# AutonomousVehicleLaboratory/vision_semantic_segmentation

Measured on AMD Instinct MI355X. Metric: fused frames/sec/GPU (1920x1080 + 120k pts) + max|dlog-odds| vs ref, higher is better.
Workload: dtype f16 hi+lo split, MX-FP4 correction passes, fp32 accumulate

## Files before the change

include/avl_hip.h:

```cpp
#ifndef AVL_HIP_H
#define AVL_HIP_H

#include <stdint.h>

#ifdef __cplusplus
extern "C" {
#endif

#define AVL_OK 0
#define AVL_E_ARG (-1)
#define AVL_E_HIP (-2)
#define AVL_E_UNSUPPORTED (-3)

#define AVL_F32 0
#define AVL_F64 1
#define AVL_BF16 2
#define AVL_F16 3

#define AVL_MAX_MAP_CLASSES 16

const char* avl_version(void);
int avl_last_error(char* buf, int len);


// ... 290 lines not shown
#define AVL_OP_SUBSAMPLE 10
#define AVL_OP_DWPW 11

#define AVL_OP_BOTTLENECK 12

typedef struct avl_seg_op {
    int32_t kind;
    int32_t dtype;
    const void* in;
    const void* in2;
    void* out;
    const void* weight;
    const float* bias;
    int32_t in_h, in_w, in_c, in_ld, in_rows;
    int32_t out_h, out_w, out_c, out_ld, out_rows;
    int32_t in2_ld;
    int32_t ksize, stride, pad, dil, groups;
    int32_t relu;
    int32_t out_f32;
    int32_t w_rows;
    int32_t w_layout;
    int32_t w_split;
    int32_t mx_flags;
    const void* in_lo;
    const void* in2_lo;
    void* out_lo;
    const void* w_mx;
    const void* in_mx;
    void* out_mx;
    const void* in2_mx;
    const void* in3;
    const void* in3_mx;
    int32_t in3_c, in3_ld;
    int32_t batch;
    int32_t bias_per_image;
    int32_t in_format;
    int32_t raw_batch;
    void* out2;
    void* out2_lo;
    int32_t out2_ld, n_split;
} avl_seg_op;

#define AVL_IN_U8_HWC 0
#define AVL_IN_F32_CHW 1

#define AVL_MX_IN_LO 1
#define AVL_MX_RES_LO 2
#define AVL_MX_OUT_LO 4

typedef struct avl_seg_plan avl_seg_plan;

int avl_seg_plan_create(const avl_seg_op* ops_host, int n_ops, avl_seg_plan** out_plan);
void avl_seg_plan_destroy(avl_seg_plan* plan);
int avl_seg_plan_run(avl_seg_plan* plan, void* stream);
int avl_seg_plan_capture(avl_seg_plan* plan, void* stream);
int avl_seg_plan_profile(avl_seg_plan* plan, void* stream, float* ms_host, double* flops_host, double* bytes_host);
int avl_seg_plan_num_ops(const avl_seg_plan* plan);
int avl_seg_plan_nonfinite(avl_seg_plan* plan, void* stream, unsigned long long* counts_host);

#define AVL_GEMM_PLAIN 0
#define AVL_GEMM_RING 1
#define AVL_GEMM_RING_MX 2
#define AVL_GEMM_MX_PIPE 3

typedef struct avl_gemm_route {
    int32_t kernel;
    int32_t dtype;
    int32_t tile_m, tile_n;
    int32_t wm, wn;
    int32_t mi;
    int32_t stages;
    int32_t nsub;
    int32_t io;
    int32_t ast;
    int32_t ext;
    int32_t late;
    int32_t launches;
    int32_t m_tiles, n_tiles;
    int32_t workgroups;
} avl_gemm_route;

int avl_seg_gemm_route(const avl_seg_op* op, avl_gemm_route* out);

#ifdef __cplusplus
}
#endif
#endif
```

vision_semantic_segmentation_amd/csrc/seg_conv.hip:

```cpp
#include "seg_types.h"
#include "seg_preprocess.h"

namespace avl {
namespace {

constexpr int kThreads = 256;

template <typename T, bool F32IN = false>
__global__ void __launch_bounds__(kThreads) k_stem(const unsigned char* __restrict__ img, int H, int W,
                                                  const float* __restrict__ w, const float* __restrict__ bias,
                                                  T* __restrict__ out, int OH, int OW, int out_ld) {
    const int idx = blockIdx.x * kThreads + threadIdx.x;
    if (idx >= OH * OW) return;
    img = image_base(img, (long long)H * W, F32IN ? 3 * (int)sizeof(float) : 3);
    out = image_base(out, (long long)OH * OW, out_ld);
    const int oy = idx / OW, ox = idx % OW;
    float acc[64];
#pragma unroll
    for (int c = 0; c < 64; ++c) acc[c] = bias[c];
    const float mean[3] = {0.485f, 0.456f, 0.406f}, stdv[3] = {0.229f, 0.224f, 0.225f};
    for (int ky = 0; ky < 7; ++ky) {
        const int iy = oy * 2 - 3 + ky;
        for (int kx = 0; kx < 7; ++kx) {
            const int ix = ox * 2 - 3 + kx;
// ... 358 lines not shown
    }
}

template <typename T>
__global__ void __launch_bounds__(kThreads) k_dwconv_split(const T* __restrict__ in, const T* __restrict__ in_lo, const float* __restrict__ w,
                                                          const float* __restrict__ bias, T* __restrict__ out, T* __restrict__ out_lo,
                                                          int H, int W, int C, int in_ld, int OH, int OW, int out_ld, int pad, int dil, int relu) {
    const int c8n = C / 8;
    const long long idx = (long long)blockIdx.x * kThreads + threadIdx.x;
    if (idx >= (long long)OH * OW * c8n) return;
    in = image_base(in, (long long)H * W, in_ld);
    in_lo = image_base(in_lo, (long long)H * W, in_ld);
    out = image_base(out, (long long)OH * OW, out_ld);
    out_lo = image_base(out_lo, (long long)OH * OW, out_ld);
    const int c8 = (int)(idx % c8n);
    const int pix = (int)(idx / c8n), oy = pix / OW, ox = pix % OW;
    float acc[8];
    {
        const float4 b0 = *reinterpret_cast<const float4*>(bias + c8 * 8), b1 = *reinterpret_cast<const float4*>(bias + c8 * 8 + 4);
        acc[0] = b0.x; acc[1] = b0.y; acc[2] = b0.z; acc[3] = b0.w; acc[4] = b1.x; acc[5] = b1.y; acc[6] = b1.z; acc[7] = b1.w;
    }
    float xv[9][8];
    bool ok[9];
#pragma unroll
    for (int t = 0; t < 9; ++t) {
        const int iy = oy - pad + (t / 3) * dil, ix = ox - pad + (t % 3) * dil;
        ok[t] = iy >= 0 && iy < H && ix >= 0 && ix < W;
        const long long o = ok[t] ? ((long long)iy * W + ix) * in_ld + c8 * 8 : (long long)c8 * 8;
        Vec8<T>::load(in + o, xv[t]);
        if (in_lo) {
            float l[8];
            Vec8<T>::load(in_lo + o, l);
#pragma unroll
            for (int i = 0; i < 8; ++i) xv[t][i] += l[i];
        }
    }
#pragma unroll
    for (int t = 0; t < 9; ++t) {
        const float4 w0 = *reinterpret_cast<const float4*>(w + t * C + c8 * 8), w1 = *reinterpret_cast<const float4*>(w + t * C + c8 * 8 + 4);
        const float wt[8] = {w0.x, w0.y, w0.z, w0.w, w1.x, w1.y, w1.z, w1.w};
#pragma unroll
        for (int i = 0; i < 8; ++i) acc[i] = fmaf(ok[t] ? xv[t][i] : 0.f, wt[i], acc[i]);
    }
    if (relu) {
#pragma unroll
        for (int i = 0; i < 8; ++i) acc[i] = fmaxf(acc[i], 0.f);
    }
    Vec8<T>::store(out + (long long)pix * out_ld + c8 * 8, acc);
    if (out_lo) {
#pragma unroll
        for (int i = 0; i < 8; ++i) acc[i] -= to_f32(from_f32<T>(acc[i]));
        Vec8<T>::store(out_lo + (long long)pix * out_ld + c8 * 8, acc);
    }
}

template <typename T>
__global__ void __launch_bounds__(kThreads) k_gap_partial(const T* __restrict__ in, int M, int C, int in_ld,
                                                         float* __restrict__ partial) {
    const int c8n = C / 8;
    const int G = gridDim.x;
    in = image_base(in, M, in_ld);
    partial = image_base(partial, G, C);
    for (int c8 = threadIdx.x; c8 < c8n; c8 += kThreads) {
        float s[8] = {0, 0, 0, 0, 0, 0, 0, 0};
        int r = blockIdx.x;
        for (; r + 3 * G < M; r += 4 * G) {
            float v0[8], v1[8], v2[8], v3[8];
            Vec8<T>::load(in + (long long)r * in_ld + c8 * 8, v0);
            Vec8<T>::load(in + (long long)(r + G) * in_ld + c8 * 8, v1);
            Vec8<T>::load(in + (long long)(r + 2 * G) * in_ld + c8 * 8, v2);
            Vec8<T>::load(in + (long long)(r + 3 * G) * in_ld + c8 * 8, v3);
#pragma unroll
            for (int i = 0; i < 8; ++i) s[i] += (v0[i] + v1[i]) + (v2[i] + v3[i]);
        }
        for (; r < M; r += G) {
            float v[8];
            Vec8<T>::load(in + (long long)r * in_ld + c8 * 8, v);
#pragma unroll
            for (int i = 0; i < 8; ++i) s[i] += v[i];
        }
        Vec8<float>::store(partial + (long long)blockIdx.x * C + c8 * 8, s);
    }
}
__global__ void __launch_bounds__(kThreads) k_gap_final(const float* __restrict__ partial, int G, int C, int M,
                                                       float* __restrict__ out, int out_ld) {
    __shared__ float red[8][32];
    const int cl = threadIdx.x & 31, sl = threadIdx.x >> 5;
    const int c = blockIdx.x * 32 + cl;
    partial = image_base(partial, G, C);
    out = image_base(out, 1, out_ld);
    float s = 0.f;
    if (c < C)
        for (int g = sl; g < G; g += 8) s += partial[(long long)g * C + c];
    red[sl][cl] = s;
    __syncthreads();
    if (sl == 0 && c < C) {
        float t = 0.f;
#pragma unroll
        for (int k = 0; k < 8; ++k) t += red[k][cl];
        out[c] = t / (float)M;
    }
}

__global__ void __launch_bounds__(kThreads) k_gemv(const float* __restrict__ in, const float* __restrict__ w,
                                                  const float* __restrict__ bias, float* __restrict__ out, int N, int K, int relu,
                                                  int in_ld, int out_ld) {
    const int n = blockIdx.x * (kThreads / 64) + (threadIdx.x >> 6);
    const int lane = threadIdx.x & 63;
    if (n >= N) return;
    in = image_base(in, 1, in_ld);
    out = image_base(out, 1, out_ld);
    const float* wr = w + (long long)n * K;
    float s0 = 0.f, s1 = 0.f, s2 = 0.f, s3 = 0.f;
    if ((K & 3) == 0 && (reinterpret_cast<uintptr_t>(wr) & 15) == 0 && (reinterpret_cast<uintptr_t>(in) & 15) == 0) {
#pragma unroll 8
        for (int k = lane * 4; k < K; k += 256) {
            const float4 a = *reinterpret_cast<const float4*>(wr + k), b = *reinterpret_cast<const float4*>(in + k);
            s0 = fmaf(a.x, b.x, s0); s1 = fmaf(a.y, b.y, s1); s2 = fmaf(a.z, b.z, s2); s3 = fmaf(a.w, b.w, s3);
        }
    } else {
        for (int k = lane; k < K; k += 64) s0 = fmaf(wr[k], in[k], s0);
    }
    float s = (s0 + s1) + (s2 + s3);
#pragma unroll
    for (int off = 32; off > 0; off >>= 1) s += __shfl_down(s, off);
    if (lane == 0) {
        s += bias ? bias[n] : 0.f;
        out[n] = relu ? fmaxf(s, 0.f) : s;
    }
}

__global__ void __launch_bounds__(kThreads) k_argmax(const float* __restrict__ logits, int M, int C, int ld,
                                                    unsigned char* __restrict__ out) {
    const int m = blockIdx.x * kThreads + threadIdx.x;
    if (m >= M) return;
    const float* p = logits + (long long)m * ld;
    float best = p[0];
    int bi = 0;
    for (int c = 1; c < C; ++c) {
        const float v = p[c];
        if (v > best || (v != v && best == best)) { best = v; bi = c; }
    }
    out[m] = (unsigned char)bi;
}

template <typename T>
__global__ void __launch_bounds__(kThreads) k_subsample(const T* __restrict__ in, int W, int C, int in_ld,
                                                       T* __restrict__ out, int H, int OH, int OW, int out_ld, int stride) {
    const int c8n = C / 8;
    const long long idx = (long long)blockIdx.x * kThreads + threadIdx.x;
    if (idx >= (long long)OH * OW * c8n) return;
    in = image_base(in, (long long)H * W, in_ld);
    out = image_base(out, (long long)OH * OW, out_ld);
    const int c8 = (int)(idx % c8n);
    const int pix = (int)(idx / c8n), oy = pix / OW, ox = pix % OW;
    float v[8];
    Vec8<T>::load(in + ((long long)(oy * stride) * W + ox * stride) * in_ld + c8 * 8, v);
    Vec8<T>::store(out + (long long)pix * out_ld + c8 * 8, v);
}

__global__ void __launch_bounds__(kThreads) k_preprocess(const unsigned char* __restrict__ bgr, int H, int W, PreParams q,
                                                        unsigned char* __restrict__ out, int OH, int OW) {
    const int idx = blockIdx.x * kThreads + threadIdx.x;
    if (idx >= OH * OW) return;
    int v[3];
    preprocessed_rgb(bgr, H, W, q.cam, q.factor, idx % OW, idx / OW, v);
#pragma unroll
    for (int c = 0; c < 3; ++c) out[3ll * idx + c] = (unsigned char)v[c];
}

struct AreaAxis { int s1, s2; float w_first, w_mid, w_last; };
__device__ __forceinline__ AreaAxis area_axis(int d, double scale, int ssize) {
    const double f1 = d * scale, f2 = f1 + scale;
    const double cell = fmin(scale, (double)ssize - f1);
    int s1 = (int)ceil(f1), s2 = (int)floor(f2);
    s2 = min(s2, ssize - 1);
// ... 46 lines not shown
                break;
            }
            hipLaunchKernelGGL(k_stem<T>, dim3(blocks_for((long long)op.out_h * op.out_w), 1, nimg), dim3(kThreads), 0, s,
                               static_cast<const unsigned char*>(op.in), op.in_h, op.in_w, w, op.bias, out, op.out_h, op.out_w,
                               op.out_ld);
            break;
        case AVL_OP_MAXPOOL:
            hipLaunchKernelGGL(k_maxpool<T>, dim3(blocks_for((long long)op.out_h * op.out_w * (op.in_c / 8)), 1, nimg), dim3(kThreads), 0, s,
                               in, op.in_h, op.in_w, op.in_c, op.in_ld, out, op.out_h, op.out_w, op.out_ld, static_cast<const T*>(op.in_lo),
                               static_cast<T*>(op.out_lo));
            break;
        case AVL_OP_GCONV: {
            const int cg = op.in_c / op.groups;
            const dim3 grid(blocks_for((long long)op.out_h * op.out_w), op.groups, nimg);
#define AVL_GCONV(CG)                                                                                                   \
    hipLaunchKernelGGL((k_gconv<T, CG>), grid, dim3(kThreads), 0, s, in, op.in_h, op.in_w, op.in_ld, w, op.bias, out, \
                       op.out_h, op.out_w, op.out_ld, op.stride, op.dil)
            if (cg == 4) AVL_GCONV(4);
            else if (cg == 8) AVL_GCONV(8);
            else if (cg == 16) AVL_GCONV(16);
            else if (cg == 32) AVL_GCONV(32);
            else if (cg == 2) AVL_GCONV(2);
            else return set_error(AVL_E_UNSUPPORTED, "grouped conv with %d channels per group", cg);
#undef AVL_GCONV
            break;
        }
        case AVL_OP_DWCONV: {
            if (op.ksize != 3) return launch_dwconv_k(op, s);
            if ((op.in_lo == nullptr) != (op.out_lo == nullptr) && !op.out_mx) {
                hipLaunchKernelGGL(k_dwconv_split<T>, dim3(blocks_for((long long)op.out_h * op.out_w * (op.in_c / 8)), 1, nimg), dim3(kThreads), 0, s,
                                   in, static_cast<const T*>(op.in_lo), w, op.bias, out, static_cast<T*>(op.out_lo), op.in_h, op.in_w,
                                   op.in_c, op.in_ld, op.out_h, op.out_w, op.out_ld, op.pad, op.dil, op.relu);
                break;
            }
            DwGeom g;
            g.H = op.in_h; g.W = op.in_w; g.C = op.in_c; g.in_ld = op.in_ld; g.OH = op.out_h; g.OW = op.out_w; g.out_ld = op.out_ld;
            g.pad = op.pad; g.dil = op.dil; g.relu = op.relu;
            g.gh = (op.out_h + op.dil - 1) / op.dil;
            g.gw = (op.out_w + op.dil - 1) / op.dil;
            const int chunks = op.in_c / 8;
            g.nchunk = chunks < 64 ? chunks : 64;
            while (chunks % g.nchunk) --g.nchunk;
            g.cl = kThreads / g.nchunk;
            g.cgroups = chunks / g.nchunk;
            const long long combs = (long long)op.dil * op.dil;
            g.band_w = g.gw; g.band_h = g.gh;
            if (op.dil == 1) {
                g.band_w = 2 * g.cl < g.gw ? 2 * g.cl : g.gw;
                g.band_h = g.gh < 16 ? g.gh : 16;
                const int nbx = (g.gw + g.band_w - 1) / g.band_w;
                while (g.band_h > 4 && (long long)g.cgroups * nbx * ((g.gh + g.band_h - 1) / g.band_h) < 512) g.band_h = (g.band_h + 1) / 2;
            }
            g.nbx = (g.gw + g.band_w - 1) / g.band_w;
            g.nby = (g.gh + g.band_h - 1) / g.band_h;
            g.units = (int)(combs * g.nby * g.nbx);
            const int target = 32 * g.cl, unit_px = g.band_h * g.band_w;
            g.upb = (op.dil == 1 || unit_px >= target) ? 1 : (target + unit_px - 1) / unit_px;
            const unsigned nblk = (unsigned)((g.units + g.upb - 1) / g.upb) * g.cgroups;
            if constexpr (sizeof(T) == 2) {
                if (op.in_lo && (op.out_lo || op.out_mx)) {
                    MxOut mx;
                    memset(&mx, 0, sizeof(mx));
                    if (op.out_mx) {
                        const auto o = mx_bundle(op.out_mx, op.out_rows, op.out_c);
                        mx.q[0] = o.q[0]; mx.s[0] = o.s[0];
                        if (op.out_lo || (op.mx_flags & AVL_MX_OUT_LO)) { mx.q[1] = o.q[1]; mx.s[1] = o.s[1]; }
                        mx.srows = o.srows; mx.ldq = o.ldq;
                    }
                    hipLaunchKernelGGL((k_dwconv<T, true>), dim3(nblk, 1, nimg), dim3(kThreads), 0, s, in, w, op.bias, out,
                                       static_cast<const T*>(op.in2), g, static_cast<const T*>(op.in_lo), static_cast<T*>(op.out_lo), mx);
                    break;
                }
            }
            hipLaunchKernelGGL((k_dwconv<T, false>), dim3(nblk, 1, nimg), dim3(kThreads), 0, s, in, w, op.bias, out,
                               static_cast<const T*>(op.in2), g, static_cast<const T*>(nullptr), static_cast<T*>(nullptr), MxOut());
            break;
        }
        case AVL_OP_BILINEAR:
            hipLaunchKernelGGL(k_bilinear<T>, dim3(blocks_for((long long)op.out_h * op.out_w * (op.in_c / 8)), 1, nimg), dim3(kThreads), 0, s,
                               in, static_cast<const T*>(op.in_lo), op.in_h, op.in_w, op.in_c, op.in_ld, out, static_cast<T*>(op.out_lo),
                               op.out_h, op.out_w, op.out_ld);
            break;
        case AVL_OP_GAP: {
            const int G = 256;
            float* partial = static_cast<float*>(const_cast<void*>(op.in2));
            hipLaunchKernelGGL(k_gap_partial<T>, dim3(G, 1, nimg), dim3(kThreads), 0, s, in, op.in_h * op.in_w, op.in_c, op.in_ld, partial);
            AVL_LAUNCH_CHECK();
            hipLaunchKernelGGL(k_gap_final, dim3((op.in_c + 31) / 32, 1, nimg), dim3(kThreads), 0, s, partial, G, op.in_c,
                               op.in_h * op.in_w, static_cast<float*>(op.out), op.out_ld);
            break;
        }
        case AVL_OP_SUBSAMPLE:
            hipLaunchKernelGGL(k_subsample<T>, dim3(blocks_for((long long)op.out_h * op.out_w * (op.in_c / 8)), 1, nimg), dim3(kThreads), 0, s,
                               in, op.in_w, op.in_c, op.in_ld, out, op.in_h, op.out_h, op.out_w, op.out_ld, op.stride);
            break;
        default:
            return set_error(AVL_E_ARG, "op kind %d is not a typed conv op", op.kind);
    }
    AVL_LAUNCH_CHECK();
    return AVL_OK;
}

}

int validate_conv_op(const avl_seg_op& op) {
    const int es = elem_size(op.dtype);
    AVL_REQUIRE(op.in && op.out, "op %d has NULL in/out", op.kind);
    AVL_REQUIRE(op.in_h > 0 && op.in_w > 0 && op.out_h > 0 && op.out_w > 0, "op %d has empty spatial dims", op.kind);
    const long long in_pix = (long long)op.in_h * op.in_w * op_batch(op), out_pix = (long long)op.out_h * op.out_w * op_batch(op);
    switch (op.kind) {
        case AVL_OP_STEM:
            if (op.in2 && op_batch(op) > 1 && !op.raw_batch)
                return set_error(AVL_E_UNSUPPORTED, "a pre-processing stem (in2 = camera block) takes one raw frame unless raw_batch = 1: batch %d",
                                 op.batch);
            AVL_REQUIRE(op.weight && op.bias && op.out_c == 64 && op.in_c == 3, "stem expects 3 -> 64 channels");
            if (op.stride == 4) {
                const int ch = (op.in_h + 6 - 7) / 2 + 1, cw = (op.in_w + 6 - 7) / 2 + 1;
                AVL_REQUIRE(is_half(op.dtype) && op.w_layout == 1, "a pooled stem (stride 4) is the MFMA kernel (16-bit, w_layout 1): dtype %d, w_layout %d",
                            op.dtype, op.w_layout);
                AVL_REQUIRE(!op.w_split && !op.out_lo, "a pooled stem (stride 4) writes one plane: w_split %d with%s out_lo", op.w_split, op.out_lo ? "" : "out");
                AVL_REQUIRE(op.out_h == (ch + 2 - 3) / 2 + 1 && op.out_w == (cw + 2 - 3) / 2 + 1, "pooled stem output size %d x %d (conv %d x %d)",
                            op.out_h, op.out_w, ch, cw);
                AVL_REQUIRE(reinterpret_cast<uintptr_t>(op.out) % 16 == 0, "pooled stem: unaligned output");
            } else
                AVL_REQUIRE(op.out_h == (op.in_h + 6 - 7) / 2 + 1 && op.out_w == (op.in_w + 6 - 7) / 2 + 1, "stem output size");
            AVL_REQUIRE(op.out_rows >= out_pix && op.out_ld >= 64 && (op.out_ld * es) % 16 == 0, "stem output buffer");
            AVL_REQUIRE(op.w_layout == 0 || (op.w_layout == 1 && is_half(op.dtype)), "stem weight layout %d", op.w_layout);
            if (op.in2) {
                AVL_REQUIRE(is_half(op.dtype) ? op.w_layout == 1 : (op.dtype == AVL_F32 && op.w_layout == 0),
                            "a pre-processing stem is the MFMA kernel (16-bit, w_layout 1) or the fp32 kernel (AVL_F32, w_layout 0): dtype %d, w_layout %d",
                            op.dtype, op.w_layout);
                AVL_REQUIRE(reinterpret_cast<uintptr_t>(op.in2) % 4 == 0, "stem camera block alignment: in2 (one block, or `batch` blocks of "
                            "AVL_STEM_CAMERA_BYTES with raw_batch) must be 4-byte aligned");
                const int nb = op_batch(op);
                AVL_REQUIRE(op.in2_ld > 0 && op.in_rows > 0 && op.in_rows % nb == 0 && (op.in_rows / nb) % op.in2_ld == 0,
                            "stem raw frame: in_rows %d is not batch %d * src_h * src_w for an integer src_h (in2_ld = src_w = %d)", op.in_rows, nb, op.in2_ld);
                const int src_w = op.in2_ld, src_h = op.in_rows / nb / op.in2_ld, f = src_w / op.in_w;
                AVL_REQUIRE(f >= 1 && op.in_w == src_w / f && op.in_h == src_h / f, "stem raw frame %dx%d does not scale to %dx%d by an integer factor",
                            src_h, src_w, op.in_h, op.in_w);
            } else {
                AVL_REQUIRE(op.in_rows >= in_pix, "stem input buffer");
            }
            return AVL_OK;
        case AVL_OP_GEMV:
            AVL_REQUIRE(op.dtype == AVL_F32, "gemv reads and writes fp32 vectors: dtype %d", op.dtype);
            AVL_REQUIRE(op.weight && op.in_c > 0 && op.out_c > 0, "gemv shapes");
            AVL_REQUIRE(op_batch(op) == 1 || (op.in_ld >= op.in_c && op.out_ld >= op.out_c), "batched gemv: vector strides in_ld %d / out_ld %d", op.in_ld, op.out_ld);
            return AVL_OK;
        case AVL_OP_ARGMAX:
            AVL_REQUIRE(op.dtype == AVL_F32, "argmax reads fp32 logits: dtype %d", op.dtype);
            AVL_REQUIRE(op.in_c > 0 && op.in_c <= 256 && op.in_ld >= op.in_c && op.in_rows >= in_pix && op.out_rows >= in_pix, "argmax shapes");
            return AVL_OK;
        case AVL_OP_GAP:
            AVL_REQUIRE(is_half(op.dtype) || op.dtype == AVL_F32, "gap dtype %d", op.dtype);
            AVL_REQUIRE(op.in2 && op.in_c % 8 == 0 && op.in_rows >= in_pix && op.in_ld >= op.in_c, "gap shapes / scratch");
            AVL_REQUIRE((op.in_ld * es) % 16 == 0, "gap in_ld");
            AVL_REQUIRE((reinterpret_cast<uintptr_t>(op.in) | reinterpret_cast<uintptr_t>(op.in2)) % 16 == 0, "gap input / scratch not 16-byte aligned");
            AVL_REQUIRE(op_batch(op) == 1 || op.out_ld >= op.in_c, "batched gap: out_ld %d", op.out_ld);
            return AVL_OK;
        default:
            break;
    }
    AVL_REQUIRE(is_half(op.dtype) || op.dtype == AVL_F32, "op %d dtype %d", op.kind, op.dtype);
    AVL_REQUIRE(op.in_c % 8 == 0 || (op.kind == AVL_OP_GCONV), "op %d: channels %d not a multiple of 8", op.kind, op.in_c);
    AVL_REQUIRE(op.in_rows >= in_pix && op.out_rows >= out_pix, "op %d: allocated rows too small", op.kind);
    AVL_REQUIRE(op.in_ld >= op.in_c && op.out_ld >= op.out_c, "op %d: leading dims", op.kind);
    AVL_REQUIRE((op.in_ld * es) % 16 == 0 && (op.out_ld * es) % 16 == 0, "op %d: row strides must be 16-byte multiples", op.kind);
    AVL_REQUIRE((reinterpret_cast<uintptr_t>(op.in) | reinterpret_cast<uintptr_t>(op.out)) % 16 == 0, "op %d: unaligned buffers", op.kind);
    if (op.out_mx && op.kind == AVL_OP_DWCONV && op.ksize == 3) {
        AVL_REQUIRE(op.dtype == AVL_F16 && op.in_lo && op.out_c % 256 == 0 && op.out_ld == op.out_c && (op.in_c / 8) % 4 == 0,
                    "dwconv: out_mx needs the split f16 form, channels %% 256 == 0 and a dense output");
// ... 95 lines not shown
```

vision_semantic_segmentation_amd/csrc/seg_stem_mfma.hip:

```cpp
#include "seg_types.h"
#include "seg_preprocess.h"

namespace avl {
namespace {

constexpr int S_TH = 8, S_TW = 32;
constexpr int ROW = 224;

template <typename HT>
struct StemArgs {
    const unsigned char* img;
    const HT* w;
    const float* bias;
    HT* out;
    HT* out_lo;
    int H, W, OH, OW, out_ld, tiles_x;
    int PH, PW;
    const PreCamera* cam;
    int srcH, srcW, factor;
};

template <typename HT, bool PRE, bool SPLIT = false, bool F32IN = false, bool POOL = false>
__global__ void __launch_bounds__(256) k_stem_mfma(StemArgs<HT> p) {
    typedef typename Half16<HT>::v8 v8;
// ... 168 lines not shown
                } else {
#pragma unroll
                    for (int i = 0; i < 8; ++i) al[i] = (HT)0.f;
                }
#pragma unroll
                for (int nj = 0; nj < 4; ++nj) {
                    const v8 wl = *reinterpret_cast<const v8*>(p.w + 4 * 6 * 16 * 32 + ((nj * 6 + st) * 16 + fr) * 32 + kq * 8);
                    acc[nj] = Half16<HT>::mfma(wf[nj][st], al, acc[nj]);
                    acc[nj] = Half16<HT>::mfma(wl, a, acc[nj]);
                }
            }
        }
        if constexpr (POOL) {
            if (sub * 16 + fr < NPOS) {
                float lo[8], hi[8];
#pragma unroll
                for (int r = 0; r < 4; ++r) {
                    lo[r] = fmaxf(acc[0][r] + bias[r], 0.f);
                    lo[4 + r] = fmaxf(acc[1][r] + bias[4 + r], 0.f);
                    hi[r] = fmaxf(acc[2][r] + bias[8 + r], 0.f);
                    hi[4 + r] = fmaxf(acc[3][r] + bias[12 + r], 0.f);
                }
                const int pos = sy * CTW + sx;
                HT* sp = stage + pos * 64;
                Vec8<HT>::store(sp + (((kq * 2) ^ (pos & 7)) << 3), lo);
                Vec8<HT>::store(sp + (((kq * 2 + 1) ^ (pos & 7)) << 3), hi);
            }
            continue;
        }
        const int oy = oy0 + sy, ox = ox0 + sx;
        if (oy < p.OH && ox < p.OW) {
            float lo[8], hi[8];
#pragma unroll
            for (int r = 0; r < 4; ++r) {
                lo[r] = fmaxf(acc[0][r] + bias[r], 0.f);
                lo[4 + r] = fmaxf(acc[1][r] + bias[4 + r], 0.f);
                hi[r] = fmaxf(acc[2][r] + bias[8 + r], 0.f);
                hi[4 + r] = fmaxf(acc[3][r] + bias[12 + r], 0.f);
            }
            HT* op = p.out + ((long long)oy * p.OW + ox) * p.out_ld + kq * 16;
            if constexpr (SPLIT) {
                float l0[8], l1[8];
#pragma unroll
                for (int r = 0; r < 8; ++r) {
                    const float h0 = (float)(HT)lo[r], h1 = (float)(HT)hi[r];
                    l0[r] = lo[r] - h0; l1[r] = hi[r] - h1;
                    lo[r] = h0; hi[r] = h1;
                }
                HT* ol = p.out_lo + ((long long)oy * p.OW + ox) * p.out_ld + kq * 16;
                Vec8<HT>::store(ol, l0);
                Vec8<HT>::store(ol + 8, l1);
            }
            Vec8<HT>::store(op, lo);
            Vec8<HT>::store(op + 8, hi);
        }
    }
    if constexpr (POOL) {
        __syncthreads();
        for (int i = tid; i < 4 * 16 * 8; i += 256) {
            const int c = i & 7, lpy = i >> 7, lpx = (i >> 3) & 15;
            const int py = ty * 4 + lpy, px = tx * 16 + lpx;
            if (py >= p.PH || px >= p.PW) continue;
            float m[8];
#pragma unroll
            for (int j = 0; j < 8; ++j) m[j] = -INFINITY;
            for (int ky = 0; ky < 3; ++ky) {
                const int cy = py * 2 - 1 + ky;
                if (cy < 0 || cy >= p.OH) continue;
                for (int kx = 0; kx < 3; ++kx) {
                    const int cx = px * 2 - 1 + kx;
                    if (cx < 0 || cx >= p.OW) continue;
                    const int pos = (lpy * 2 + ky) * CTW + lpx * 2 + kx;
                    float v[8];
                    Vec8<HT>::load(stage + pos * 64 + ((c ^ (pos & 7)) << 3), v);
#pragma unroll
                    for (int j = 0; j < 8; ++j) m[j] = fmaxf(m[j], v[j]);
                }
            }
            Vec8<HT>::store(p.out + ((long long)py * p.PW + px) * p.out_ld + c * 8, m);
        }
    }
}

}

template <typename HT>
int launch_stem_typed(const avl_seg_op& op, hipStream_t s) {
    StemArgs<HT> a;
    a.img = static_cast<const unsigned char*>(op.in);
    a.w = static_cast<const HT*>(op.weight);
    a.bias = op.bias;
    a.out = static_cast<HT*>(op.out);
    a.out_lo = static_cast<HT*>(op.out_lo);
    a.H = op.in_h; a.W = op.in_w; a.OH = op.out_h; a.OW = op.out_w; a.out_ld = op.out_ld;
    const bool pool = op.stride == 4;
    a.PH = op.out_h; a.PW = op.out_w;
    if (pool) { a.OH = (op.in_h + 6 - 7) / 2 + 1; a.OW = (op.in_w + 6 - 7) / 2 + 1; }
    a.tiles_x = pool ? (op.out_w + 15) / 16 : (op.out_w + S_TW - 1) / S_TW;
    const int tiles_y = pool ? (op.out_h + 3) / 4 : (op.out_h + S_TH - 1) / S_TH;
    a.cam = static_cast<const PreCamera*>(op.in2);
    a.srcW = op.in2_ld;
    a.srcH = op.in2_ld > 0 ? op.in_rows / op_batch(op) / op.in2_ld : 0;
    a.factor = op.in_w > 0 ? a.srcW / op.in_w : 1;
    const dim3 grid(a.tiles_x * tiles_y, 1, op_batch(op));
    if (pool) {
        if (op.in_format == AVL_IN_F32_CHW) hipLaunchKernelGGL((k_stem_mfma<HT, false, false, true, true>), grid, dim3(256), 0, s, a);
        else if (op.in2) hipLaunchKernelGGL((k_stem_mfma<HT, true, false, false, true>), grid, dim3(256), 0, s, a);
        else hipLaunchKernelGGL((k_stem_mfma<HT, false, false, false, true>), grid, dim3(256), 0, s, a);
    } else if (op.in_format == AVL_IN_F32_CHW) {
        if (op.w_split) {
            if (!op.out_lo) return set_error(AVL_E_ARG, "split stem (w_split = 1): out_lo is NULL");
            hipLaunchKernelGGL((k_stem_mfma<HT, false, true, true>), grid, dim3(256), 0, s, a);
        } else {
            hipLaunchKernelGGL((k_stem_mfma<HT, false, false, true>), grid, dim3(256), 0, s, a);
        }
    } else if (op.w_split) {
        if (!op.out_lo) return set_error(AVL_E_ARG, "split stem (w_split = 1): out_lo is NULL");
        if (op.in2)
            hipLaunchKernelGGL((k_stem_mfma<HT, true, true>), grid, dim3(256), 0, s, a);
        else
            hipLaunchKernelGGL((k_stem_mfma<HT, false, true>), dim3(a.tiles_x * tiles_y, 1, op_batch(op)), dim3(256), 0, s, a);
    } else if (op.in2)
        hipLaunchKernelGGL((k_stem_mfma<HT, true>), grid, dim3(256), 0, s, a);
    else
        hipLaunchKernelGGL((k_stem_mfma<HT, false>), dim3(a.tiles_x * tiles_y, 1, op_batch(op)), dim3(256), 0, s, a);
    AVL_LAUNCH_CHECK();
    return AVL_OK;
}

int launch_stem_mfma(const avl_seg_op& op, hipStream_t s) {
    return op.dtype == AVL_F16 ? launch_stem_typed<f16>(op, s) : launch_stem_typed<bf16>(op, s);
}

}
```

vision_semantic_segmentation_amd/network.py:

```python
import collections
import ctypes as C
import hashlib
import math

import numpy as np
import torch

from . import _lib

BN_EPS = 1e-5

OP_STEM, OP_MAXPOOL, OP_GEMM, OP_GCONV, OP_DWCONV, OP_BILINEAR, OP_GAP, OP_GEMV, OP_ARGMAX, OP_SUBSAMPLE, OP_DWPW, OP_BOTTLENECK = range(1, 13)
OP_NAMES = {1: "stem", 2: "maxpool", 3: "gemm", 4: "gconv", 5: "dwconv", 6: "bilinear", 7: "gap", 8: "gemv", 9: "argmax", 10: "subsample", 11: "dwpw",
            12: "bottleneck"}


class AvlSegOp(C.Structure):
    _fields_ = [
        ("kind", C.c_int32), ("dtype", C.c_int32),
        ("in_", C.c_void_p), ("in2", C.c_void_p), ("out", C.c_void_p), ("weight", C.c_void_p), ("bias", C.c_void_p),
        ("in_h", C.c_int32), ("in_w", C.c_int32), ("in_c", C.c_int32), ("in_ld", C.c_int32), ("in_rows", C.c_int32),
        ("out_h", C.c_int32), ("out_w", C.c_int32), ("out_c", C.c_int32), ("out_ld", C.c_int32), ("out_rows", C.c_int32),
        ("in2_ld", C.c_int32),
        ("ksize", C.c_int32), ("stride", C.c_int32), ("pad", C.c_int32), ("dil", C.c_int32), ("groups", C.c_int32),
        ("relu", C.c_int32), ("out_f32", C.c_int32), ("w_rows", C.c_int32), ("w_layout", C.c_int32), ("w_split", C.c_int32), ("mx_flags", C.c_int32),
        ("in_lo", C.c_void_p), ("in2_lo", C.c_void_p), ("out_lo", C.c_void_p),
        ("w_mx", C.c_void_p), ("in_mx", C.c_void_p), ("out_mx", C.c_void_p), ("in2_mx", C.c_void_p),
        ("in3", C.c_void_p), ("in3_mx", C.c_void_p), ("in3_c", C.c_int32), ("in3_ld", C.c_int32),
        ("batch", C.c_int32), ("bias_per_image", C.c_int32),
        ("in_format", C.c_int32),
        ("raw_batch", C.c_int32),
        ("out2", C.c_void_p), ("out2_lo", C.c_void_p), ("out2_ld", C.c_int32), ("n_split", C.c_int32),
    ]


AVL_IN_U8_HWC, AVL_IN_F32_CHW = 0, 1
INPUT_FORMATS = {"u8_hwc": AVL_IN_U8_HWC, "f32_nchw": AVL_IN_F32_CHW}


AVL_MX_IN_LO, AVL_MX_RES_LO, AVL_MX_OUT_LO = 1, 2, 4


GEMM_KERNELS = ("k_gemm", "k_gemm_ring", "k_gemm_ring_mx", "k_gemm_mx_pipe")


class AvlGemmRoute(C.Structure):
    _fields_ = [(name, C.c_int32) for name in (
        "kernel", "dtype", "tile_m", "tile_n", "wm", "wn", "mi", "stages", "nsub", "io", "ast", "ext", "late",
        "launches", "m_tiles", "n_tiles", "workgroups")]


def gemm_route(op):
    r = AvlGemmRoute()
    _lib.check(_lib.lib().avl_seg_gemm_route(C.byref(op), C.byref(r)), "avl_seg_gemm_route")
    d = {name: getattr(r, name) for name, _ in AvlGemmRoute._fields_}
    d["kernel"] = GEMM_KERNELS[r.kernel]
    return d


def gemm_kernel_name(route):
    t = {_lib.AVL_F32: "float", _lib.AVL_BF16: "bf16", _lib.AVL_F16: "f16"}[route["dtype"]]
    args = {"k_gemm": [t, "wm", "wn"],
            "k_gemm_ring": [t, "wm", "wn", "mi", "stages", "nsub", "io", "ast", "true" if route["ext"] else "false"],
            "k_gemm_ring_mx": ["io", "mi"],
            "k_gemm_mx_pipe": ["io", "mi", "late"]}[route["kernel"]]
    return "%s<%s>" % (route["kernel"], ", ".join(str(route.get(a, a)) for a in args))


_vp, _i = C.c_void_p, C.c_int
_lib._register_seg({
    "avl_seg_gemm_route": (_i, [C.POINTER(AvlSegOp), C.POINTER(AvlGemmRoute)]),
    "avl_seg_plan_create": (_i, [C.POINTER(AvlSegOp), _i, C.POINTER(C.c_void_p)]),
    "avl_seg_plan_destroy": (None, [_vp]),
    "avl_seg_plan_run": (_i, [_vp, _vp]),
    "avl_seg_plan_capture": (_i, [_vp, _vp]),
    "avl_seg_plan_profile": (_i, [_vp, _vp, _vp, _vp, _vp]),
    "avl_seg_plan_num_ops": (_i, [_vp]),
    "avl_seg_plan_nonfinite": (_i, [_vp, _vp, _vp]),
})


PLANES = (64, 128, 256, 512)
EXPANSION = 4
BACKBONES = {
    "resnet50": ((3, 4, 6, 3), 1, 64),
    "resnet101": ((3, 4, 23, 3), 1, 64),
    "resnet152": ((3, 8, 36, 3), 1, 64),
    "resnext50_32x4d": ((3, 4, 6, 3), 32, 4),
    "resnext101_32x8d": ((3, 4, 23, 3), 32, 8),
    "wide_resnet50_2": ((3, 4, 6, 3), 1, 128),
    "wide_resnet101_2": ((3, 4, 23, 3), 1, 128),
}
DEFAULT_BACKBONE = "resnext50_32x4d"
UNBUILDABLE_BACKBONES = ("ResNet", "resnet18", "resnet34")
LAYERS, GROUPS, WIDTH_PER_GROUP = BACKBONES[DEFAULT_BACKBONE]


def backbone_arch(name):
    if name in BACKBONES:
        return BACKBONES[name]
    if name in UNBUILDABLE_BACKBONES:
        raise NotImplementedError("MODEL.BACKBONE %r is a BasicBlock ResNet: the reference's MyResNet (backbone/resnet.py:17-18) "
                                  "hard-codes 2048 output and 256 low-level channels, so it cannot build either; supported: %s"
                                  % (name, ", ".join(sorted(BACKBONES))))
    raise NotImplementedError("MODEL.BACKBONE %r is not supported; supported: %s" % (name, ", ".join(sorted(BACKBONES))))


REFINE_KERNEL_SIZES = (1, 2, 3, 4, 5, 6, 7)


def refine_kernel_sizes(refine_kernel_size, refine_channels):
    n = len(refine_channels)
    if refine_kernel_size is None:
        return (3,) * n
    ks = tuple(int(k) for k in refine_kernel_size)
    if len(ks) != n:
        if all(k == 3 for k in ks):
            return (3,) * n
        raise ValueError("MODEL.DECODER.REFINE_KERNEL_SIZE %s has %d entries, REFINE_CHANNELS %d: one kernel size per refine block "
                         "(decoder.py:20)" % (list(ks), len(ks), n))
    bad = [k for k in ks if k not in REFINE_KERNEL_SIZES]
    if bad:
        raise ValueError("MODEL.DECODER.REFINE_KERNEL_SIZE %s: depthwise kernels are built for sizes %s" % (list(ks), ", ".join(map(str, REFINE_KERNEL_SIZES))))
    return ks


def _bn_keys(prefix, c):
    return [(prefix + ".weight", (c,)), (prefix + ".bias", (c,)), (prefix + ".running_mean", (c,)),
            (prefix + ".running_var", (c,))]


def state_spec(num_classes=19, in_channels=3, aspp_out=256, atrous_channels=(256, 256, 256, 256), low_level_out=256,
               refine_channels=(256, 256), backbone=DEFAULT_BACKBONE, refine_kernel_size=None):
    refine_kernel_size = refine_kernel_sizes(refine_kernel_size, refine_channels)
    layers, groups, wpg = backbone_arch(backbone)
    spec = [("backbone.conv1.weight", (64, in_channels, 7, 7))] + _bn_keys("backbone.bn1", 64)
    inplanes = 64
    for li, (planes, nblocks) in enumerate(zip(PLANES, layers), start=1):
        width = int(planes * (wpg / 64.0)) * groups
        for b in range(nblocks):
            p = "backbone.layer%d.%d" % (li, b)
            spec += [(p + ".conv1.weight", (width, inplanes, 1, 1))] + _bn_keys(p + ".bn1", width)
            spec += [(p + ".conv2.weight", (width, width // groups, 3, 3))] + _bn_keys(p + ".bn2", width)
            spec += [(p + ".conv3.weight", (planes * EXPANSION, width, 1, 1))] + _bn_keys(p + ".bn3", planes * EXPANSION)
            if b == 0:
                spec += [(p + ".downsample.0.weight", (planes * EXPANSION, inplanes, 1, 1))] + _bn_keys(p + ".downsample.1", planes * EXPANSION)
            inplanes = planes * EXPANSION
    feat, low = inplanes, PLANES[0] * EXPANSION
    spec += [("aspp.module_pyramid.0.conv.weight", (atrous_channels[0], feat, 1, 1))] + _bn_keys("aspp.module_pyramid.0.bn", atrous_channels[0])
    for i in range(1, len(atrous_channels)):
        p = "aspp.module_pyramid.%d" % i
        spec += [(p + ".depthwise_cnn.conv.weight", (feat, 1, 3, 3))] + _bn_keys(p + ".depthwise_cnn.bn", feat)
        spec += [(p + ".pointwise_cnn.conv.weight", (atrous_channels[i], feat, 1, 1))] + _bn_keys(p + ".pointwise_cnn.bn", atrous_channels[i])
    spec += [("aspp.global_avg_pool.1.conv.weight", (256, feat, 1, 1))] + _bn_keys("aspp.global_avg_pool.1.bn", 256)
# ... 1115 lines not shown
```

Before: 234.6.

## Add persistent stem+maxpool kernel with prefetched word loads and XCD-aware tiles

Adds a persistent fused stem-conv + maxpool kernel for uint8 HWC input that is word-aligned. Each workgroup loops over tiles in an XCD-contiguous order, keeps the stem weights in registers, and uses an LDS lookup table for normalisation. It prefetches the next tile's 32-bit image words into registers while the current tile's MFMA and pool work runs. The GAP final reduction is also unrolled with a fixed partial count. The aim is to cut per-tile launch and setup overhead and hide global load latency, at the cost of more code and more register/LDS pressure.

```diff
diff --git a/include/avl_hip.h b/include/avl_hip.h
--- a/include/avl_hip.h
+++ b/include/avl_hip.h
@@ -396,6 +396,15 @@
 
 int avl_seg_gemm_route(const avl_seg_op* op, avl_gemm_route* out);
 
+typedef struct avl_stem_pool_route_t {
+    int32_t word_path;
+    int32_t tiles_x, tiles_y, tiles;
+    int32_t slots;
+    int32_t grid;
+    int32_t lds_bytes;
+} avl_stem_pool_route_t;
+int avl_stem_pool_route(const void* img, int in_h, int in_w, int dtype, int slots, avl_stem_pool_route_t* out);
+
 #ifdef __cplusplus
 }
 #endif
diff --git a/vision_semantic_segmentation_amd/csrc/seg_conv.hip b/vision_semantic_segmentation_amd/csrc/seg_conv.hip
--- a/vision_semantic_segmentation_amd/csrc/seg_conv.hip
+++ b/vision_semantic_segmentation_amd/csrc/seg_conv.hip
@@ -464,16 +464,22 @@
         Vec8<float>::store(partial + (long long)blockIdx.x * C + c8 * 8, s);
     }
 }
-__global__ void __launch_bounds__(kThreads) k_gap_final(const float* __restrict__ partial, int G, int C, int M,
+constexpr int kGapG = 256;
+__global__ void __launch_bounds__(kThreads) k_gap_final(const float* __restrict__ partial, int C, int M,
                                                        float* __restrict__ out, int out_ld) {
     __shared__ float red[8][32];
     const int cl = threadIdx.x & 31, sl = threadIdx.x >> 5;
     const int c = blockIdx.x * 32 + cl;
-    partial = image_base(partial, G, C);
+    partial = image_base(partial, kGapG, C);
     out = image_base(out, 1, out_ld);
     float s = 0.f;
-    if (c < C)
-        for (int g = sl; g < G; g += 8) s += partial[(long long)g * C + c];
+    if (c < C) {
+        float v[kGapG / 8];
+#pragma unroll
+        for (int i = 0; i < kGapG / 8; ++i) v[i] = partial[(long long)(sl + 8 * i) * C + c];
+#pragma unroll
+        for (int i = 0; i < kGapG / 8; ++i) s += v[i];
+    }
     red[sl][cl] = s;
     __syncthreads();
     if (sl == 0 && c < C) {
@@ -686,11 +692,11 @@
                                op.out_h, op.out_w, op.out_ld);
             break;
         case AVL_OP_GAP: {
-            const int G = 256;
+            const int G = kGapG;
             float* partial = static_cast<float*>(const_cast<void*>(op.in2));
             hipLaunchKernelGGL(k_gap_partial<T>, dim3(G, 1, nimg), dim3(kThreads), 0, s, in, op.in_h * op.in_w, op.in_c, op.in_ld, partial);
             AVL_LAUNCH_CHECK();
-            hipLaunchKernelGGL(k_gap_final, dim3((op.in_c + 31) / 32, 1, nimg), dim3(kThreads), 0, s, partial, G, op.in_c,
+            hipLaunchKernelGGL(k_gap_final, dim3((op.in_c + 31) / 32, 1, nimg), dim3(kThreads), 0, s, partial, op.in_c,
                                op.in_h * op.in_w, static_cast<float*>(op.out), op.out_ld);
             break;
         }
diff --git a/vision_semantic_segmentation_amd/csrc/seg_stem_mfma.hip b/vision_semantic_segmentation_amd/csrc/seg_stem_mfma.hip
--- a/vision_semantic_segmentation_amd/csrc/seg_stem_mfma.hip
+++ b/vision_semantic_segmentation_amd/csrc/seg_stem_mfma.hip
@@ -274,6 +274,182 @@
     }
 }
 
+constexpr int PS_CTH = 9, PS_CTW = 33, PS_ITH = 2 * PS_CTH + 5, PS_ITW = 2 * PS_CTW + 5;
+constexpr int PS_NPOS = PS_CTH * PS_CTW, PS_NSUBT = (PS_NPOS + 15) / 16;
+constexpr int PS_WORDS = 54;
+constexpr int PS_RPW = (PS_ITH + 3) / 4;
+constexpr int PS_LDS_BYTES = ((PS_ITH + 1) * ROW + PS_NPOS * 64 + 3 * 256) * 2 + 64 * 4;
+static_assert(4 * (PS_WORDS - 1) - 1 < PS_ITW * 3 && 4 * PS_WORDS - 1 >= PS_ITW * 3 && 4 * PS_WORDS <= ROW, "54 words cover the 213 bytes and stay in the row");
+
+template <typename HT>
+__global__ void __launch_bounds__(256, 3) k_stem_pool_persist(StemArgs<HT> p, int tiles) {
+    typedef typename Half16<HT>::v8 v8;
+    constexpr int CTW = PS_CTW, ITH = PS_ITH, ITW = PS_ITW, NPOS = PS_NPOS, NSUBT = PS_NSUBT;
+    __shared__ __attribute__((aligned(16))) HT tile[(ITH + 1) * ROW];
+    __shared__ __attribute__((aligned(16))) HT stage[NPOS * 64];
+    __shared__ HT lut[3 * 256];
+    __shared__ __attribute__((aligned(16))) float sbias[64];
+    const int tid = threadIdx.x, lane = tid & 63;
+    const int wave = __builtin_amdgcn_readfirstlane(tid >> 6);
+    p.img = image_base(p.img, (long long)p.H * p.W, 3);
+    p.out = image_base(p.out, (long long)p.PH * p.PW, p.out_ld);
+    int t;
+    {
+        const int bid = blockIdx.x, nwg = gridDim.x, xcd = bid & 7, local = bid >> 3, qq = nwg >> 3, r = nwg & 7;
+        t = (xcd < r ? xcd * (qq + 1) : r * (qq + 1) + (xcd - r) * qq) + local;
+    }
+    const uint32_t* img32 = reinterpret_cast<const uint32_t*>(p.img);
+    const int wpr = p.W * 3 / 4;
+    uint32_t wd[PS_RPW];
+    auto tile_load = [&](int tt) {
+        const int tx = tt % p.tiles_x, ty = tt / p.tiles_x;
+        const int wc = min(max(tx * 48 - 4 + lane, 0), wpr - 1);
+#pragma unroll
+        for (int k = 0; k < PS_RPW; ++k) {
+            const int cy = min(max(ty * 16 - 5 + wave + 4 * k, 0), p.H - 1);
+            wd[k] = img32[(long long)cy * wpr + wc];
+        }
+    };
+    const int c0 = lane % 3;
+    auto tile_convert = [&](int tt) {
+        const int tx = tt % p.tiles_x, ty = tt / p.tiles_x;
+        const int w0 = tx * 48 - 4 + lane;
+        const bool wok = lane < PS_WORDS && w0 >= 0 && w0 < wpr, wok1 = lane + 1 < PS_WORDS && w0 + 1 >= 0 && w0 + 1 < wpr;
+        uint32_t nw[PS_RPW];
+#pragma unroll
+        for (int k = 0; k < PS_RPW; ++k) nw[k] = (uint32_t)__shfl_down((int)wd[k], 1);
+#pragma unroll
+        for (int k = 0; k < PS_RPW; ++k) {
+            const int ly = wave + 4 * k, iy = ty * 16 - 5 + ly;
+            const bool rok = iy >= 0 && iy < p.H;
+            unsigned h[4];
+#pragma unroll
+            for (int i = 0; i < 4; ++i) {
+                const unsigned b = i < 3 ? (wd[k] >> (8 * i + 8)) & 255u : nw[k] & 255u;
+                const HT v = lut[((c0 + i) % 3) * 256 + b];
+                h[i] = rok && (i < 3 ? wok : wok1) && 4 * lane + i < ITW * 3 ? __builtin_bit_cast(unsigned short, v) : 0u;
+            }
+            if (lane < PS_WORDS && ly < ITH)
+                *reinterpret_cast<uint2*>(tile + ly * ROW + 4 * lane) = make_uint2(h[0] | (h[1] << 16), h[2] | (h[3] << 16));
+        }
+    };
+
+    if (t < tiles) tile_load(t);
+    const int fr = lane & 15, kq = lane >> 4;
+    v8 wf[4][6];
+#pragma unroll
+    for (int nj = 0; nj < 4; ++nj)
+#pragma unroll
+        for (int st = 0; st < 6; ++st)
+            wf[nj][st] = *reinterpret_cast<const v8*>(p.w + ((nj * 6 + st) * 16 + fr) * 32 + kq * 8);
+    if (tid < 64) sbias[tid] = p.bias[tid];
+    {
+        const float mean[3] = {0.485f, 0.456f, 0.406f}, stdv[3] = {0.229f, 0.224f, 0.225f};
+#pragma unroll
+        for (int ci = 0; ci < 3; ++ci) {
+            const float v = ((float)tid / 255.0f - mean[ci]) / stdv[ci];
+            lut[ci * 256 + tid] = (HT)v;
+        }
+    }
+    for (int e = tid; e < (ITH + 1) * ROW; e += 256) {
+        const int ly = e / ROW, lc = e - ly * ROW;
+        if (ly >= ITH || lc >= ITW * 3) tile[e] = (HT)0.f;
+    }
+    __builtin_amdgcn_s_waitcnt(0x0F70);
+    __syncthreads();
+
+    for (; t < tiles; t += gridDim.x) {
+        const int tx = t % p.tiles_x, ty = t / p.tiles_x;
+        tile_convert(t);
+        __syncthreads();
+        if (t + (int)gridDim.x < tiles) tile_load(t + gridDim.x);
+
+        for (int sub = wave; sub < NSUBT; sub += 4) {
+            const int pos = min(sub * 16 + fr, NPOS - 1);
+            const int sy = pos / CTW, sx = pos - sy * CTW;
+            f32x4 acc[4];
+#pragma unroll
+            for (int nj = 0; nj < 4; ++nj) acc[nj] = f32x4{0.f, 0.f, 0.f, 0.f};
+#pragma unroll
+            for (int st = 0; st < 6; ++st) {
+                const int q = st * 4 + kq;
+                const int ky = q / 3, piece = q - ky * 3;
+                v8 a;
+                if (q < 21) {
+                    const uint32_t* src = reinterpret_cast<const uint32_t*>(tile + (sy * 2 + ky) * ROW + sx * 6 + piece * 8);
+                    uint32_t u[4] = {src[0], src[1], src[2], src[3]};
+                    __builtin_memcpy(&a, u, 16);
+                } else {
+#pragma unroll
+                    for (int i = 0; i < 8; ++i) a[i] = (HT)0.f;
+                }
+#pragma unroll
+                for (int nj = 0; nj < 4; ++nj) acc[nj] = Half16<HT>::mfma(wf[nj][st], a, acc[nj]);
+            }
+            if (sub * 16 + fr < NPOS) {
+                float bias[16], lo[8], hi[8];
+#pragma unroll
+                for (int j = 0; j < 4; ++j) {
+                    const float4 b = *reinterpret_cast<const float4*>(sbias + kq * 16 + 4 * j);
+                    bias[4 * j] = b.x; bias[4 * j + 1] = b.y; bias[4 * j + 2] = b.z; bias[4 * j + 3] = b.w;
+                }
+#pragma unroll
+                for (int r = 0; r < 4; ++r) {
+                    lo[r] = fmaxf(acc[0][r] + bias[r], 0.f);
+                    lo[4 + r] = fmaxf(acc[1][r] + bias[4 + r], 0.f);
+                    hi[r] = fmaxf(acc[2][r] + bias[8 + r], 0.f);
+                    hi[4 + r] = fmaxf(acc[3][r] + bias[12 + r], 0.f);
+                }
+                HT* sp = stage + pos * 64;
+                Vec8<HT>::store(sp + (((kq * 2) ^ (pos & 7)) << 3), lo);
+                Vec8<HT>::store(sp + (((kq * 2 + 1) ^ (pos & 7)) << 3), hi);
+            }
+        }
+        __syncthreads();
+        for (int i = tid; i < 4 * 16 * 8; i += 256) {
+            const int c = i & 7, lpy = i >> 7, lpx = (i >> 3) & 15;
+            const int py = ty * 4 + lpy, px = tx * 16 + lpx;
+            if (py >= p.PH || px >= p.PW) continue;
+            float m[8];
+#pragma unroll
+            for (int j = 0; j < 8; ++j) m[j] = -INFINITY;
+            for (int ky = 0; ky < 3; ++ky) {
+                const int cy = py * 2 - 1 + ky;
+                if (cy < 0 || cy >= p.OH) continue;
+                for (int kx = 0; kx < 3; ++kx) {
+                    const int cx = px * 2 - 1 + kx;
+                    if (cx < 0 || cx >= p.OW) continue;
+                    const int pos = (lpy * 2 + ky) * CTW + lpx * 2 + kx;
+                    float v[8];
+                    Vec8<HT>::load(stage + pos * 64 + ((c ^ (pos & 7)) << 3), v);
+#pragma unroll
+                    for (int j = 0; j < 8; ++j) m[j] = fmaxf(m[j], v[j]);
+                }
+            }
+            Vec8<HT>::store(p.out + ((long long)py * p.PW + px) * p.out_ld + c * 8, m);
+        }
+    }
+}
+
+}
+
+static bool stem_pool_word_path(const void* img, int W) {
+    return (reinterpret_cast<uintptr_t>(img) & 3) == 0 && (3LL * W) % 4 == 0;
+}
+static int stem_pool_grid(int tiles, int slots) { return tiles < slots ? tiles : slots; }
+
+template <typename HT>
+static int stem_pool_slots() {
+    static int n = 0;
+    if (n == 0) {
+        int dev = 0, per_cu = 0;
+        hipDeviceProp_t prop;
+        if (hipGetDevice(&dev) == hipSuccess && hipGetDeviceProperties(&prop, dev) == hipSuccess &&
+            hipOccupancyMaxActiveBlocksPerMultiprocessor(&per_cu, k_stem_pool_persist<HT>, 256, 0) == hipSuccess && per_cu > 0)
+            n = per_cu * prop.multiProcessorCount;
+        if (n <= 0) n = 256;
+    }
+    return n;
 }
 
 template <typename HT>
@@ -298,7 +474,10 @@
     if (pool) {
         if (op.in_format == AVL_IN_F32_CHW) hipLaunchKernelGGL((k_stem_mfma<HT, false, false, true, true>), grid, dim3(256), 0, s, a);
         else if (op.in2) hipLaunchKernelGGL((k_stem_mfma<HT, true, false, false, true>), grid, dim3(256), 0, s, a);
-        else hipLaunchKernelGGL((k_stem_mfma<HT, false, false, false, true>), grid, dim3(256), 0, s, a);
+        else if (stem_pool_word_path(a.img, a.W)) {
+            const int tiles = a.tiles_x * tiles_y;
+            hipLaunchKernelGGL(k_stem_pool_persist<HT>, dim3(stem_pool_grid(tiles, stem_pool_slots<HT>()), 1, op_batch(op)), dim3(256), 0, s, a, tiles);
+        } else hipLaunchKernelGGL((k_stem_mfma<HT, false, false, false, true>), grid, dim3(256), 0, s, a);
     } else if (op.in_format == AVL_IN_F32_CHW) {
         if (op.w_split) {
             if (!op.out_lo) return set_error(AVL_E_ARG, "split stem (w_split = 1): out_lo is NULL");
@@ -325,3 +504,19 @@
 }
 
 }
+
+extern "C" int avl_stem_pool_route(const void* img, int in_h, int in_w, int dtype, int slots, avl_stem_pool_route_t* out) {
+    AVL_REQUIRE(out, "avl_stem_pool_route: out is NULL");
+    AVL_REQUIRE(in_h > 0 && in_w > 0, "avl_stem_pool_route: frame %d x %d", in_h, in_w);
+    AVL_REQUIRE(dtype == AVL_F16 || dtype == AVL_BF16, "avl_stem_pool_route: dtype %d is not a 16-bit type", dtype);
+    const int oh = (in_h + 6 - 7) / 2 + 1, ow = (in_w + 6 - 7) / 2 + 1;
+    const int ph = (oh + 2 - 3) / 2 + 1, pw = (ow + 2 - 3) / 2 + 1;
+    out->word_path = avl::stem_pool_word_path(img, in_w) ? 1 : 0;
+    out->tiles_x = (pw + 15) / 16;
+    out->tiles_y = (ph + 3) / 4;
+    out->tiles = out->tiles_x * out->tiles_y;
+    out->slots = slots > 0 ? slots : dtype == AVL_F16 ? avl::stem_pool_slots<avl::f16>() : avl::stem_pool_slots<avl::bf16>();
+    out->grid = out->word_path ? avl::stem_pool_grid(out->tiles, out->slots) : out->tiles;
+    out->lds_bytes = avl::PS_LDS_BYTES;
+    return AVL_OK;
+}
diff --git a/vision_semantic_segmentation_amd/network.py b/vision_semantic_segmentation_amd/network.py
--- a/vision_semantic_segmentation_amd/network.py
+++ b/vision_semantic_segmentation_amd/network.py
@@ -67,9 +67,20 @@
     return "%s<%s>" % (route["kernel"], ", ".join(str(route.get(a, a)) for a in args))
 
 
+class AvlStemPoolRoute(C.Structure):
+    _fields_ = [(name, C.c_int32) for name in ("word_path", "tiles_x", "tiles_y", "tiles", "slots", "grid", "lds_bytes")]
+
+
+def stem_pool_route(address, h, w, dtype=_lib.AVL_F16, slots=0):
+    r = AvlStemPoolRoute()
+    _lib.check(_lib.lib().avl_stem_pool_route(C.c_void_p(address), h, w, dtype, slots, C.byref(r)), "avl_stem_pool_route")
+    return {name: getattr(r, name) for name, _ in AvlStemPoolRoute._fields_}
+
+
 _vp, _i = C.c_void_p, C.c_int
 _lib._register_seg({
     "avl_seg_gemm_route": (_i, [C.POINTER(AvlSegOp), C.POINTER(AvlGemmRoute)]),
+    "avl_stem_pool_route": (_i, [_vp, _i, _i, _i, _i, C.POINTER(AvlStemPoolRoute)]),
     "avl_seg_plan_create": (_i, [C.POINTER(AvlSegOp), _i, C.POINTER(C.c_void_p)]),
     "avl_seg_plan_destroy": (None, [_vp]),
     "avl_seg_plan_run": (_i, [_vp, _vp]),
```

After: 235.7 (median of 5 runs). About the same (+0.5%).
